# databricks/spark-deep-learning

Measured on AMD Instinct MI355X. Metric: images/sec, higher is better.
Workload: dtype bf16; 1 GPU; model=resnet50, global_batch=512, image=224, parallelism=dp1

## Files before the change

sparkdl/ops/csrc/batchnorm.hip:

```cpp

#include "common.hip.h"
#include "kernels.h"

namespace {

constexpr int kBlock = 256;
constexpr int kVec = 8;


__device__ __forceinline__ void bn_block_fold(
    float* lds_a, float* lds_b, const float* a, const float* b,
    int lane_col, int cols, float* out_a, float* out_b) {
  for (int c = threadIdx.x; c < cols; c += kBlock) {
    lds_a[c] = 0.f;
    lds_b[c] = 0.f;
  }
  __syncthreads();
#pragma unroll
  for (int j = 0; j < kVec; ++j) {
    atomicAdd(&lds_a[lane_col + j], a[j]);
    atomicAdd(&lds_b[lane_col + j], b[j]);
  }
  __syncthreads();
  for (int c = threadIdx.x; c < cols; c += kBlock) {
    atomicAdd(&out_a[c], lds_a[c]);
    atomicAdd(&out_b[c], lds_b[c]);
  }
}

__global__ __launch_bounds__(kBlock) void bn_stats_k(
    const short* __restrict__ x, float* __restrict__ scratch,
    long long rows, int cols) {
  __shared__ float lds[2 * 2048];
  const int tpr = cols / kVec;
  const int rpb = kBlock / min(tpr, kBlock);
  const int lane_col = (threadIdx.x % tpr) * kVec;
  const int row_off = threadIdx.x / tpr;

  float s[kVec] = {0.f}, ss[kVec] = {0.f};
  if (row_off < rpb) {
    for (long long r = (long long)blockIdx.x * rpb + row_off; r < rows;
         r += (long long)gridDim.x * rpb) {
      const short8 v = *(const short8*)(x + r * cols + lane_col);
#pragma unroll
      for (int j = 0; j < kVec; ++j) {
        const float f = bf2f(v[j]);
        s[j] += f;
        ss[j] += f * f;
      }
    }
  }
  bn_block_fold(lds, lds + cols, s, ss, lane_col, cols, scratch,
                scratch + cols);
}

__global__ void bn_finalize_k(
    const float* __restrict__ scratch, const float* __restrict__ gamma,
    const float* __restrict__ beta, float* __restrict__ running_mean,
    float* __restrict__ running_var, float* __restrict__ save_mean,
    float* __restrict__ save_rstd, float* __restrict__ scale,
    float* __restrict__ shift, long long rows, int cols, float momentum,
    float eps, int training) {
  const int c = blockIdx.x * blockDim.x + threadIdx.x;
  if (c >= cols) return;
  float mean, rstd;
  if (training) {
    mean = scratch[c] / rows;
    const float var = fmaxf(scratch[cols + c] / rows - mean * mean, 0.f);
    rstd = rsqrtf(var + eps);
    const float unbiased = rows > 1 ? var * rows / (rows - 1) : var;
    running_mean[c] += momentum * (mean - running_mean[c]);
    running_var[c] += momentum * (unbiased - running_var[c]);
    save_mean[c] = mean;
    save_rstd[c] = rstd;
  } else {
    mean = running_mean[c];
    rstd = rsqrtf(running_var[c] + eps);
    save_mean[c] = mean;
    save_rstd[c] = rstd;
  }
  const float sc = gamma[c] * rstd;
  scale[c] = sc;
  shift[c] = beta[c] - mean * sc;
}

template <bool RELU, bool RES>
__global__ __launch_bounds__(kBlock) void bn_apply_k(
    const short* __restrict__ x, const short* __restrict__ res,
    const float* __restrict__ scale, const float* __restrict__ shift,
    short* __restrict__ y, unsigned char* __restrict__ mask,
    long long rows, int cols) {
  const int tpr = cols / kVec;
  const int rpb = kBlock / min(tpr, kBlock);
  const int lane_col = (threadIdx.x % tpr) * kVec;
  const int row_off = threadIdx.x / tpr;
  if (row_off >= rpb) return;
  const float4v sc0 = *(const float4v*)(scale + lane_col);
  const float4v sc1 = *(const float4v*)(scale + lane_col + 4);
  const float4v sh0 = *(const float4v*)(shift + lane_col);
  const float4v sh1 = *(const float4v*)(shift + lane_col + 4);

  for (long long r = (long long)blockIdx.x * rpb + row_off; r < rows;
       r += (long long)gridDim.x * rpb) {
    const long long base = r * cols + lane_col;
    const short8 v = *(const short8*)(x + base);
    short8 o;
    unsigned char mbits = 0;
#pragma unroll
    for (int j = 0; j < kVec; ++j) {
      float f = bf2f(v[j]) * (j < 4 ? sc0[j] : sc1[j - 4]) +
                (j < 4 ? sh0[j] : sh1[j - 4]);
      if (RES) f += bf2f(res[base + j]);
      if (RELU) {
        if (f > 0.f) mbits |= (unsigned char)(1u << j);
        f = fmaxf(f, 0.f);
      }
      o[j] = f2bf(f);
    }
    *(short8*)(y + base) = o;
    if (RELU) mask[(r * cols + lane_col) / kVec] = mbits;
  }
}


template <bool RELU>
__global__ __launch_bounds__(kBlock) void bn_bwd_reduce_k(
    const short* __restrict__ x, const unsigned char* __restrict__ mask,
    const short* __restrict__ dy, const float* __restrict__ save_mean,
    const float* __restrict__ save_rstd, float* __restrict__ scratch,
    long long rows, int cols) {
  __shared__ float lds[2 * 2048];
  const int tpr = cols / kVec;
  const int rpb = kBlock / min(tpr, kBlock);
  const int lane_col = (threadIdx.x % tpr) * kVec;
  const int row_off = threadIdx.x / tpr;

  float s1[kVec] = {0.f}, s2[kVec] = {0.f};
  if (row_off < rpb) {
    const float4v m0 = *(const float4v*)(save_mean + lane_col);
    const float4v m1 = *(const float4v*)(save_mean + lane_col + 4);
    const float4v r0 = *(const float4v*)(save_rstd + lane_col);
    const float4v r1 = *(const float4v*)(save_rstd + lane_col + 4);
    for (long long r = (long long)blockIdx.x * rpb + row_off; r < rows;
         r += (long long)gridDim.x * rpb) {
      const long long base = r * cols + lane_col;
      const short8 xv = *(const short8*)(x + base);
      const short8 dv = *(const short8*)(dy + base);
      unsigned char mbits = 0xffu;
      if (RELU) mbits = mask[base / kVec];
#pragma unroll
      for (int j = 0; j < kVec; ++j) {
        float d = bf2f(dv[j]);
        if (RELU && !(mbits & (1u << j))) d = 0.f;
        const float mean = j < 4 ? m0[j] : m1[j - 4];
        const float rstd = j < 4 ? r0[j] : r1[j - 4];
        const float xh = (bf2f(xv[j]) - mean) * rstd;
        s1[j] += d;
        s2[j] += d * xh;
      }
    }
  }
  bn_block_fold(lds, lds + cols, s1, s2, lane_col, cols, scratch,
                scratch + cols);
}

__global__ void bn_bwd_finalize_k(
    const float* __restrict__ scratch, const float* __restrict__ gamma,
    const float* __restrict__ save_rstd, float* __restrict__ dgamma,
    float* __restrict__ dbeta, float* __restrict__ c1,
    float* __restrict__ c2, float* __restrict__ c3, long long rows,
    int cols, int training) {
  const int c = blockIdx.x * blockDim.x + threadIdx.x;
  if (c >= cols) return;
  const float sum_dym = scratch[c];
  const float sum_dymxh = scratch[cols + c];
  dgamma[c] = sum_dymxh;
  dbeta[c] = sum_dym;
  c1[c] = gamma[c] * save_rstd[c];
  if (training) {
    c2[c] = sum_dym / rows;
    c3[c] = sum_dymxh / rows;
  } else {
    c2[c] = 0.f;
    c3[c] = 0.f;
  }
}

template <bool RELU, bool RES>
__global__ __launch_bounds__(kBlock) void bn_bwd_apply_k(
    const short* __restrict__ x, const unsigned char* __restrict__ mask,
    const short* __restrict__ dy, const float* __restrict__ save_mean,
    const float* __restrict__ save_rstd, const float* __restrict__ c1,
    const float* __restrict__ c2, const float* __restrict__ c3,
    short* __restrict__ dx, short* __restrict__ dres, long long rows,
    int cols) {
  const int tpr = cols / kVec;
  const int rpb = kBlock / min(tpr, kBlock);
  const int lane_col = (threadIdx.x % tpr) * kVec;
  const int row_off = threadIdx.x / tpr;
  if (row_off >= rpb) return;
  const float4v m0 = *(const float4v*)(save_mean + lane_col);
  const float4v m1 = *(const float4v*)(save_mean + lane_col + 4);
  const float4v r0 = *(const float4v*)(save_rstd + lane_col);
  const float4v r1 = *(const float4v*)(save_rstd + lane_col + 4);
  const float4v a0 = *(const float4v*)(c1 + lane_col);
  const float4v a1 = *(const float4v*)(c1 + lane_col + 4);
  const float4v b0 = *(const float4v*)(c2 + lane_col);
  const float4v b1 = *(const float4v*)(c2 + lane_col + 4);
  const float4v g0 = *(const float4v*)(c3 + lane_col);
  const float4v g1 = *(const float4v*)(c3 + lane_col + 4);

  for (long long r = (long long)blockIdx.x * rpb + row_off; r < rows;
       r += (long long)gridDim.x * rpb) {
    const long long base = r * cols + lane_col;
    const short8 xv = *(const short8*)(x + base);
    const short8 dv = *(const short8*)(dy + base);
    unsigned char mbits = 0xffu;
    if (RELU) mbits = mask[base / kVec];
    short8 odx, odr;
#pragma unroll
    for (int j = 0; j < kVec; ++j) {
      float d = bf2f(dv[j]);
      if (RELU && !(mbits & (1u << j))) d = 0.f;
      const float mean = j < 4 ? m0[j] : m1[j - 4];
      const float rstd = j < 4 ? r0[j] : r1[j - 4];
      const float xh = (bf2f(xv[j]) - mean) * rstd;
      const float k1 = j < 4 ? a0[j] : a1[j - 4];
      const float k2 = j < 4 ? b0[j] : b1[j - 4];
      const float k3 = j < 4 ? g0[j] : g1[j - 4];
      odx[j] = f2bf(k1 * (d - k2 - xh * k3));
      if (RES) odr[j] = f2bf(d);
    }
    *(short8*)(dx + base) = odx;
    if (RES) *(short8*)(dres + base) = odr;
  }
}

int bn_grid(long long rows, int cols) {
  const int tpr = cols / kVec;
  const int rpb = kBlock / min(tpr, kBlock);
  long long blocks = (rows + rpb - 1) / rpb;
  return (int)min(blocks, 2048LL);
}

}

void launch_bn_fwd(const short* x, const short* res, const float* gamma,
                   const float* beta, float* running_mean,
                   float* running_var, float* save_mean, float* save_rstd,
                   float* scratch, short* y, unsigned char* mask,
                   long long rows, int cols, float momentum, float eps,
                   bool training, bool relu, hipStream_t stream) {
  const int grid = bn_grid(rows, cols);
  if (training)
    hipLaunchKernelGGL(bn_stats_k, dim3(grid), dim3(kBlock), 0, stream, x,
                       scratch, rows, cols);
  float* scale = scratch + 2 * cols;
  float* shift = scratch + 3 * cols;
  hipLaunchKernelGGL(bn_finalize_k, dim3((cols + 255) / 256), dim3(256), 0,
                     stream, scratch, gamma, beta, running_mean,
                     running_var, save_mean, save_rstd, scale, shift, rows,
                     cols, momentum, eps, (int)training);
  auto ap = relu ? (res ? bn_apply_k<true, true> : bn_apply_k<true, false>)
                 : (res ? bn_apply_k<false, true>
                        : bn_apply_k<false, false>);
  hipLaunchKernelGGL(ap, dim3(grid), dim3(kBlock), 0, stream, x, res,
                     scale, shift, y, mask, rows, cols);
}

void launch_bn_bwd(const short* x, const unsigned char* mask,
                   const short* dy, const float* gamma,
                   const float* save_mean, const float* save_rstd,
                   float* scratch, float* dgamma, float* dbeta, short* dx,
                   short* dres, long long rows, int cols, bool training,
                   bool relu, hipStream_t stream) {
  const int grid = bn_grid(rows, cols);
  auto rk = relu ? bn_bwd_reduce_k<true> : bn_bwd_reduce_k<false>;
  hipLaunchKernelGGL(rk, dim3(grid), dim3(kBlock), 0, stream, x, mask, dy,
                     save_mean, save_rstd, scratch, rows, cols);
  float* c1 = scratch + 2 * cols;
  float* c2 = scratch + 3 * cols;
  float* c3 = scratch + 4 * cols;
  hipLaunchKernelGGL(bn_bwd_finalize_k, dim3((cols + 255) / 256), dim3(256),
                     0, stream, scratch, gamma, save_rstd, dgamma, dbeta,
                     c1, c2, c3, rows, cols, (int)training);
  auto ak = relu ? (dres ? bn_bwd_apply_k<true, true>
                         : bn_bwd_apply_k<true, false>)
                 : (dres ? bn_bwd_apply_k<false, true>
                         : bn_bwd_apply_k<false, false>);
  hipLaunchKernelGGL(ak, dim3(grid), dim3(kBlock), 0, stream, x, mask, dy,
                     save_mean, save_rstd, c1, c2, c3, dx, dres, rows,
                     cols);
}
```

sparkdl/ops/csrc/bindings.cpp:

```cpp

#include <torch/extension.h>
#include <ATen/hip/impl/HIPStreamMasqueradingAsCUDA.h>
#include <ATen/hip/impl/HIPGuardImplMasqueradingAsCUDA.h>

#include <cmath>
#include <vector>

#include "kernels.h"

namespace {

using DeviceGuard = c10::hip::HIPGuardMasqueradingAsCUDA;

hipStream_t cur_stream() {
  return c10::hip::getCurrentHIPStreamMasqueradingAsCUDA().stream();
}

#define CHECK_BF16_CUDA(t)                                            \
  TORCH_CHECK((t).is_cuda(), #t " must be on GPU");                   \
  TORCH_CHECK((t).scalar_type() == at::kBFloat16, #t " must be bf16");\
  TORCH_CHECK((t).is_contiguous(), #t " must be contiguous")

#define CHECK_F32_CUDA(t)                                             \
  TORCH_CHECK((t).is_cuda(), #t " must be on GPU");                   \
  TORCH_CHECK((t).scalar_type() == at::kFloat, #t " must be fp32");   \
  TORCH_CHECK((t).is_contiguous(), #t " must be contiguous")

const short* bf_ptr(const at::Tensor& t) {
  return reinterpret_cast<const short*>(t.data_ptr<at::BFloat16>());
}
short* bf_ptr_mut(at::Tensor& t) {
  return reinterpret_cast<short*>(t.data_ptr<at::BFloat16>());
}


void fused_adamw_(const at::Tensor& chunks_blob, const at::Tensor& bmap,
                  int64_t nblocks, double lr, double beta1, double beta2,
                  double eps, double weight_decay, at::Tensor step_counter,
                  at::Tensor coeffs) {
  TORCH_CHECK(chunks_blob.is_cuda() && bmap.is_cuda());
  TORCH_CHECK(step_counter.is_cuda() &&
              step_counter.scalar_type() == at::kLong);
  TORCH_CHECK(coeffs.is_cuda() && coeffs.scalar_type() == at::kFloat &&
              coeffs.numel() >= 2);
  DeviceGuard guard(chunks_blob.device());
  launch_fused_adamw(
      reinterpret_cast<const TensorChunk*>(chunks_blob.data_ptr()),
      reinterpret_cast<const int2*>(bmap.data_ptr()), (int)nblocks,
      (float)lr, (float)beta1, (float)beta2, (float)eps,
      (float)weight_decay,
      reinterpret_cast<long long*>(step_counter.data_ptr<int64_t>()),
      coeffs.data_ptr<float>(), cur_stream());
}

void zero_grads_(const at::Tensor& chunks_blob, const at::Tensor& bmap,
                 int64_t nblocks) {
  TORCH_CHECK(chunks_blob.is_cuda() && bmap.is_cuda());
  DeviceGuard guard(chunks_blob.device());
  launch_zero_grads(
      reinterpret_cast<const TensorChunk*>(chunks_blob.data_ptr()),
      reinterpret_cast<const int2*>(bmap.data_ptr()), (int)nblocks,
      cur_stream());
}

void fused_sgd_(const at::Tensor& chunks_blob, const at::Tensor& bmap,
                int64_t nblocks, double lr, double momentum,
                double weight_decay, bool nesterov, bool first_step) {
  TORCH_CHECK(chunks_blob.is_cuda() && bmap.is_cuda());
  DeviceGuard guard(chunks_blob.device());
  launch_fused_sgd(
      reinterpret_cast<const TensorChunk*>(chunks_blob.data_ptr()),
      reinterpret_cast<const int2*>(bmap.data_ptr()), (int)nblocks,
      (float)lr, (float)momentum, (float)weight_decay, nesterov,
      first_step, cur_stream());
}


std::vector<at::Tensor> layernorm_fwd(const at::Tensor& x,
                                      const at::Tensor& gamma,
                                      const at::Tensor& beta, double eps) {
  CHECK_BF16_CUDA(x);
  CHECK_F32_CUDA(gamma);
  CHECK_F32_CUDA(beta);
  DeviceGuard guard(x.device());
  const int cols = (int)x.size(-1);
  const int rows = (int)(x.numel() / cols);
  TORCH_CHECK(gamma.numel() == cols && beta.numel() == cols);

  auto y = at::empty_like(x);
  auto f32 = x.options().dtype(at::kFloat);
  auto mean = at::empty({rows}, f32);
  auto rstd = at::empty({rows}, f32);
  launch_layernorm_fwd(bf_ptr(x), gamma.data_ptr<float>(),
                       beta.data_ptr<float>(), bf_ptr_mut(y),
                       mean.data_ptr<float>(), rstd.data_ptr<float>(),
                       rows, cols, (float)eps, cur_stream());
  return {y, mean, rstd};
}

std::vector<at::Tensor> layernorm_bwd(const at::Tensor& x,
                                      const at::Tensor& dy,
                                      const at::Tensor& gamma,
                                      const at::Tensor& mean,
                                      const at::Tensor& rstd) {
  CHECK_BF16_CUDA(x);
  CHECK_BF16_CUDA(dy);
  CHECK_F32_CUDA(gamma);
  DeviceGuard guard(x.device());
  const int cols = (int)x.size(-1);
  const int rows = (int)(x.numel() / cols);
  TORCH_CHECK(cols <= 8192, "layernorm_bwd LDS partials support cols<=8192");

  auto dx = at::empty_like(x);
  auto f32 = x.options().dtype(at::kFloat);
  const int blocks = layernorm_bwd_part_rows(rows);
  const int ws_rows = blocks * 4;
  auto dgamma_part = at::empty({ws_rows, cols}, f32);
  auto dbeta_part = at::empty({ws_rows, cols}, f32);
  auto dgamma = at::zeros({cols}, f32);
  auto dbeta = at::zeros({cols}, f32);
  launch_layernorm_bwd(bf_ptr(x), bf_ptr(dy), gamma.data_ptr<float>(),
                       mean.data_ptr<float>(), rstd.data_ptr<float>(),
                       bf_ptr_mut(dx), dgamma_part.data_ptr<float>(),
                       dbeta_part.data_ptr<float>(), blocks, rows, cols,
                       cur_stream());
  launch_layernorm_reduce_parts(
      dgamma_part.data_ptr<float>(), dbeta_part.data_ptr<float>(),
      dgamma.data_ptr<float>(), dbeta.data_ptr<float>(), ws_rows, cols,
      cur_stream());
  return {dx, dgamma, dbeta};
}


std::vector<at::Tensor> bn_fwd(const at::Tensor& x,
                               const c10::optional<at::Tensor>& res,
                               const at::Tensor& gamma,
                               const at::Tensor& beta,
                               at::Tensor running_mean,
                               at::Tensor running_var, double momentum,
                               double eps, bool training, bool relu) {
  CHECK_BF16_CUDA(x);
  CHECK_F32_CUDA(gamma);
  CHECK_F32_CUDA(beta);
  DeviceGuard guard(x.device());
  const int cols = (int)x.size(-1);
  const long long rows = x.numel() / cols;
  TORCH_CHECK(cols % 8 == 0 && cols <= 2048,
              "bn_fwd requires cols%8==0 and cols<=2048 (NHWC channels)");
  const short* res_ptr = nullptr;
  if (res.has_value()) {
    CHECK_BF16_CUDA(res.value());
    TORCH_CHECK(res->sizes() == x.sizes());
    res_ptr = bf_ptr(res.value());
  }
  auto f32 = x.options().dtype(at::kFloat);
  auto y = at::empty_like(x);
  auto save_mean = at::empty({cols}, f32);
  auto save_rstd = at::empty({cols}, f32);
  auto scratch = at::zeros({5 * cols}, f32);
  at::Tensor mask;
  unsigned char* mask_ptr = nullptr;
  if (relu) {
    mask = at::empty({rows * cols / 8}, x.options().dtype(at::kByte));
    mask_ptr = mask.data_ptr<unsigned char>();
  } else {
    mask = at::empty({0}, x.options().dtype(at::kByte));
  }
  launch_bn_fwd(bf_ptr(x), res_ptr, gamma.data_ptr<float>(),
                beta.data_ptr<float>(), running_mean.data_ptr<float>(),
                running_var.data_ptr<float>(), save_mean.data_ptr<float>(),
                save_rstd.data_ptr<float>(), scratch.data_ptr<float>(),
                bf_ptr_mut(y), mask_ptr, rows, cols, (float)momentum,
                (float)eps, training, relu, cur_stream());
  return {y, save_mean, save_rstd, mask};
}

std::vector<at::Tensor> bn_bwd(const at::Tensor& x,
                               const at::Tensor& mask,
                               const at::Tensor& dy,
                               const at::Tensor& gamma,
                               const at::Tensor& save_mean,
                               const at::Tensor& save_rstd, bool training,
                               bool relu, bool needs_dres) {
  CHECK_BF16_CUDA(x);
  CHECK_BF16_CUDA(dy);
  CHECK_F32_CUDA(gamma);
  DeviceGuard guard(x.device());
  const int cols = (int)x.size(-1);
  const long long rows = x.numel() / cols;
  TORCH_CHECK(!relu || mask.numel() == rows * cols / 8,
              "relu backward needs the forward's activation mask");
  auto f32 = x.options().dtype(at::kFloat);
  auto dx = at::empty_like(x);
  auto dgamma = at::empty({cols}, f32);
  auto dbeta = at::empty({cols}, f32);
  auto scratch = at::zeros({5 * cols}, f32);
  at::Tensor dres;
  short* dres_ptr = nullptr;
  if (needs_dres) {
    dres = at::empty_like(x);
    dres_ptr = bf_ptr_mut(dres);
  }
  launch_bn_bwd(bf_ptr(x),
                relu ? mask.data_ptr<unsigned char>() : nullptr,
                bf_ptr(dy), gamma.data_ptr<float>(),
                save_mean.data_ptr<float>(), save_rstd.data_ptr<float>(),
                scratch.data_ptr<float>(), dgamma.data_ptr<float>(),
                dbeta.data_ptr<float>(), bf_ptr_mut(dx), dres_ptr, rows,
                cols, training, relu, cur_stream());
  if (needs_dres) return {dx, dgamma, dbeta, dres};
  return {dx, dgamma, dbeta};
}


at::Tensor bias_gelu_fwd(const at::Tensor& x, const at::Tensor& bias) {
  CHECK_BF16_CUDA(x);
  CHECK_F32_CUDA(bias);
  DeviceGuard guard(x.device());
  const int cols = (int)x.size(-1);
  const long long rows = x.numel() / cols;
  TORCH_CHECK(bias.numel() == cols);
  auto y = at::empty_like(x);
  launch_bias_gelu_fwd(bf_ptr(x), bias.data_ptr<float>(), bf_ptr_mut(y),
                       rows, cols, cur_stream());
  return y;
}

std::vector<at::Tensor> bias_gelu_bwd(const at::Tensor& x,
                                      const at::Tensor& bias,
                                      const at::Tensor& dy) {
  CHECK_BF16_CUDA(x);
  CHECK_BF16_CUDA(dy);
  CHECK_F32_CUDA(bias);
  DeviceGuard guard(x.device());
  const int cols = (int)x.size(-1);
  const long long rows = x.numel() / cols;
  TORCH_CHECK(cols <= 16384, "bias_gelu_bwd LDS partials support cols<=16384");
  auto dx = at::empty_like(x);
  auto dbias = at::zeros({cols}, x.options().dtype(at::kFloat));
  launch_bias_gelu_bwd(bf_ptr(x), bias.data_ptr<float>(), bf_ptr(dy),
                       bf_ptr_mut(dx), dbias.data_ptr<float>(), rows, cols,
                       cur_stream());
  return {dx, dbias};
}


std::vector<at::Tensor> gemm_bias_act(const at::Tensor& A,
                                      const at::Tensor& W,
                                      const c10::optional<at::Tensor>& bias,
                                      int64_t act, bool save_z) {
  CHECK_BF16_CUDA(A);
  CHECK_BF16_CUDA(W);
  TORCH_CHECK(A.dim() == 2 && W.dim() == 2 && A.size(1) == W.size(1));
  const int M = (int)A.size(0), K = (int)A.size(1), N = (int)W.size(0);
  TORCH_CHECK(gemm_bias_act_supported(M, N, K),
              "gemm_bias_act requires K % 64 == 0");
  const float* bias_ptr = nullptr;
  if (bias.has_value()) {
    CHECK_F32_CUDA(bias.value());
    TORCH_CHECK(bias->numel() == N);
    bias_ptr = bias->data_ptr<float>();
  }
  DeviceGuard guard(A.device());
  auto C = at::empty({M, N}, A.options());
  at::Tensor Z;
  short* z_ptr = nullptr;
  if (save_z && act != 0) {
    Z = at::empty({M, N}, A.options());
    z_ptr = bf_ptr_mut(Z);
  }
  launch_gemm_bias_act(bf_ptr(A), bf_ptr(W), bias_ptr, bf_ptr_mut(C),
                       z_ptr, M, N, K, (int)act, cur_stream());
  if (z_ptr) return {C, Z};
  return {C};
}

at::Tensor gemm_stream(const at::Tensor& A, const at::Tensor& W) {
  CHECK_BF16_CUDA(A);
  CHECK_BF16_CUDA(W);
  TORCH_CHECK(A.dim() == 2 && W.dim() == 2 && A.size(1) == W.size(1));
  const long long M = A.size(0);
  const int K = (int)A.size(1), N = (int)W.size(0);
  TORCH_CHECK(gemm_stream_supported(M, N, K),
              "gemm_stream requires K in {64,128,256} and N % 64 == 0");
  DeviceGuard guard(A.device());
  auto C = at::empty({M, N}, A.options());
  launch_gemm_stream(bf_ptr(A), bf_ptr(W), bf_ptr_mut(C), M, N, K,
                     cur_stream());
  return C;
}


static const long long* seed_ptr(const c10::optional<at::Tensor>& seed) {
  if (!seed.has_value()) return nullptr;
  TORCH_CHECK(seed->is_cuda() && seed->scalar_type() == at::kLong &&
              seed->numel() >= 1);
  return reinterpret_cast<const long long*>(seed->data_ptr<int64_t>());
}

std::vector<at::Tensor> attn_fwd(const at::Tensor& Q, const at::Tensor& K,
                                 const at::Tensor& V, double dropout_p,
                                 const c10::optional<at::Tensor>& seed) {
  CHECK_BF16_CUDA(Q);
  CHECK_BF16_CUDA(K);
  CHECK_BF16_CUDA(V);
  TORCH_CHECK(Q.dim() == 3 && Q.size(2) == 64 && Q.sizes() == K.sizes() &&
                  Q.sizes() == V.sizes(),
              "attn_fwd expects [BH, S, 64] bf16 q/k/v");
  const int BH = (int)Q.size(0), S = (int)Q.size(1);
  TORCH_CHECK(S % 64 == 0, "attn_fwd requires S % 64 == 0");
  TORCH_CHECK(dropout_p == 0.0 || seed.has_value(),
              "dropout needs a seed tensor");
  DeviceGuard guard(Q.device());
  auto O = at::empty_like(Q);
  auto LSE = at::empty({BH, S}, Q.options().dtype(at::kFloat));
  auto VT = at::empty({BH, 64, S}, Q.options());
  launch_attn_pretranspose(bf_ptr(V), bf_ptr_mut(VT), BH, S, 1, 64,
                           cur_stream());
  launch_attn_fwd(bf_ptr(Q), bf_ptr(K), bf_ptr(VT), bf_ptr_mut(O),
                  LSE.data_ptr<float>(), seed_ptr(seed), BH, S, 1, 64,
                  64, (float)dropout_p, cur_stream());
  return {O, LSE};
}

std::vector<at::Tensor> attn_fwd_packed(
    const at::Tensor& qkv, double dropout_p,
    const c10::optional<at::Tensor>& seed) {
  CHECK_BF16_CUDA(qkv);
  TORCH_CHECK(qkv.dim() == 5 && qkv.size(2) == 3 && qkv.size(4) == 64 &&
                  qkv.is_contiguous(),
              "attn_fwd_packed expects contiguous [B,S,3,H,64] bf16");
  const int B = (int)qkv.size(0), S = (int)qkv.size(1),
            H = (int)qkv.size(3);
  TORCH_CHECK(S % 64 == 0, "attn requires S % 64 == 0");
  TORCH_CHECK(dropout_p == 0.0 || seed.has_value());
  DeviceGuard guard(qkv.device());
  auto O = at::empty({B, S, H * 64}, qkv.options());
  auto LSE = at::empty({B * H, S}, qkv.options().dtype(at::kFloat));
  const short* base = bf_ptr(qkv);
  auto VT = at::empty({B * H, 64, S}, qkv.options());
  launch_attn_pretranspose(base + (long long)2 * H * 64, bf_ptr_mut(VT),
                           B * H, S, H, 3 * H * 64, cur_stream());
  launch_attn_fwd(base, base + (long long)H * 64, bf_ptr(VT),
                  bf_ptr_mut(O), LSE.data_ptr<float>(), seed_ptr(seed),
                  B * H, S, H, 3 * H * 64, H * 64, (float)dropout_p,
                  cur_stream());
  return {O, LSE};
}

std::vector<at::Tensor> attn_bwd(const at::Tensor& Q, const at::Tensor& K,
                                 const at::Tensor& V, const at::Tensor& dO,
                                 const at::Tensor& LSE,
                                 const at::Tensor& Drow, double dropout_p,
                                 const c10::optional<at::Tensor>& seed) {
  CHECK_BF16_CUDA(Q);
  CHECK_BF16_CUDA(dO);
  CHECK_F32_CUDA(LSE);
  CHECK_F32_CUDA(Drow);
  const int BH = (int)Q.size(0), S = (int)Q.size(1);
  DeviceGuard guard(Q.device());
  auto dQ = at::empty_like(Q);
  auto dK = at::empty_like(K);
  auto dV = at::empty_like(V);
  auto T3 = at::empty({3, BH, 64, S}, Q.options());
  short* qt = bf_ptr_mut(T3);
  short* dot = qt + (long long)BH * 64 * S;
  short* ktt = dot + (long long)BH * 64 * S;
  launch_attn_pretranspose(bf_ptr(Q), qt, BH, S, 1, 64, cur_stream());
  launch_attn_pretranspose(bf_ptr(dO), dot, BH, S, 1, 64, cur_stream());
  launch_attn_pretranspose(bf_ptr(K), ktt, BH, S, 1, 64, cur_stream());
  launch_attn_bwd(bf_ptr(Q), bf_ptr(K), bf_ptr(V), bf_ptr(dO), qt, dot,
                  ktt, LSE.data_ptr<float>(), Drow.data_ptr<float>(),
                  bf_ptr_mut(dQ), bf_ptr_mut(dK), bf_ptr_mut(dV),
                  seed_ptr(seed), BH, S, 1, 64, 64, 64, (float)dropout_p,
                  cur_stream());
  return {dQ, dK, dV};
}

at::Tensor attn_bwd_packed(const at::Tensor& qkv, const at::Tensor& dO,
                           const at::Tensor& LSE, const at::Tensor& Drow,
                           double dropout_p,
                           const c10::optional<at::Tensor>& seed) {
  CHECK_BF16_CUDA(qkv);
  CHECK_BF16_CUDA(dO);
  CHECK_F32_CUDA(LSE);
  CHECK_F32_CUDA(Drow);
  TORCH_CHECK(qkv.dim() == 5 && qkv.is_contiguous() &&
              dO.is_contiguous());
  const int B = (int)qkv.size(0), S = (int)qkv.size(1),
            H = (int)qkv.size(3);
  DeviceGuard guard(qkv.device());
  auto dqkv = at::empty_like(qkv);
  const short* base = bf_ptr(qkv);
  short* gbase = bf_ptr_mut(dqkv);
  const int BH = B * H;
  auto T3 = at::empty({3, BH, 64, S}, qkv.options());
  short* qt = bf_ptr_mut(T3);
  short* dot = qt + (long long)BH * 64 * S;
  short* ktt = dot + (long long)BH * 64 * S;
  launch_attn_pretranspose(base, qt, BH, S, H, 3 * H * 64, cur_stream());
  launch_attn_pretranspose(bf_ptr(dO), dot, BH, S, H, H * 64,
                           cur_stream());
  launch_attn_pretranspose(base + (long long)H * 64, ktt, BH, S, H,
                           3 * H * 64, cur_stream());
  launch_attn_bwd(base, base + (long long)H * 64,
                  base + (long long)2 * H * 64, bf_ptr(dO), qt, dot, ktt,
                  LSE.data_ptr<float>(), Drow.data_ptr<float>(), gbase,
                  gbase + (long long)H * 64,
                  gbase + (long long)2 * H * 64, seed_ptr(seed), BH, S,
                  H, 3 * H * 64, H * 64, 3 * H * 64, (float)dropout_p,
                  cur_stream());
  return dqkv;
}

at::Tensor wgrad_splitk(const at::Tensor& dZ, const at::Tensor& X) {
  CHECK_BF16_CUDA(dZ);
  CHECK_BF16_CUDA(X);
  TORCH_CHECK(dZ.dim() == 2 && X.dim() == 2 && dZ.size(0) == X.size(0));
  const long long M = dZ.size(0);
  const int N = (int)dZ.size(1), K = (int)X.size(1);
  TORCH_CHECK(wgrad_splitk_supported(M, N, K),
              "wgrad_splitk requires N%256==0, K%128==0, M%64==0");
  DeviceGuard guard(dZ.device());
  auto dW = at::empty({N, K}, dZ.options().dtype(at::kFloat));
  launch_wgrad_splitk(bf_ptr(dZ), bf_ptr(X), dW.data_ptr<float>(), M, N,
                      K, cur_stream());
  return dW;
}

at::Tensor transpose_bf16(const at::Tensor& X) {
  CHECK_BF16_CUDA(X);
  TORCH_CHECK(X.dim() == 2 && X.is_contiguous());
  DeviceGuard guard(X.device());
  const int R = (int)X.size(0), C = (int)X.size(1);
  auto Y = at::empty({C, R}, X.options());
  launch_transpose_bf16(bf_ptr(X), bf_ptr_mut(Y), R, C, cur_stream());
  return Y;
}


at::Tensor gbt_histogram(const at::Tensor& B, const at::Tensor& g,
                         const at::Tensor& h, const at::Tensor& row_list,
                         const at::Tensor& bmap, int64_t n_nodes) {
  TORCH_CHECK(B.is_cuda() && B.scalar_type() == at::kByte &&
              B.is_contiguous());
  CHECK_F32_CUDA(g);
  CHECK_F32_CUDA(h);
  TORCH_CHECK(row_list.is_cuda() && row_list.scalar_type() == at::kInt);
  TORCH_CHECK(bmap.is_cuda() && bmap.scalar_type() == at::kInt &&
              bmap.size(-1) == 4);
  DeviceGuard guard(B.device());
  const int F = (int)B.size(1);
  TORCH_CHECK(F % 8 == 0, "feature dim must be padded to a multiple of 8");
  auto hist = at::zeros({n_nodes, F, 256, 2},
                        B.options().dtype(at::kFloat));
  launch_gbt_histogram(
      B.data_ptr<unsigned char>(), g.data_ptr<float>(),
      h.data_ptr<float>(), row_list.data_ptr<int>(),
      reinterpret_cast<const int4*>(bmap.data_ptr<int>()),
      (int)(bmap.numel() / 4), F, hist.data_ptr<float>(), cur_stream());
  return hist;
}

}

PYBIND11_MODULE(TORCH_EXTENSION_NAME, m) {
  m.doc() = "sparkdl MI355X-native kernels (gfx950)";
  m.def("fused_adamw_", &fused_adamw_, "Fused multi-tensor AdamW step");
  m.def("fused_sgd_", &fused_sgd_, "Fused multi-tensor SGD step");
  m.def("zero_grads_", &zero_grads_, "Zero all grads in a chunk table");
  m.def("gemm_bias_act", &gemm_bias_act, "MFMA GEMM + bias(+GELU) (N6)");
  m.def("transpose_bf16", &transpose_bf16, "bf16 2D transpose (dgrad W^T)");
  m.def("gemm_stream", &gemm_stream,
        "Streaming tall-skinny GEMM (1x1 convs)");
  m.def("wgrad_splitk", &wgrad_splitk,
        "Split-M wgrad GEMM (tr_b16 fragment path)");
  m.def("attn_fwd", &attn_fwd, "Flash attention fwd (D=64, bf16)");
  m.def("attn_bwd", &attn_bwd, "Flash attention bwd (dQ/dK/dV)");
  m.def("attn_fwd_packed", &attn_fwd_packed,
        "Flash attention fwd over the packed qkv buffer");
  m.def("attn_bwd_packed", &attn_bwd_packed,
        "Flash attention bwd -> packed dqkv");
  m.def("gbt_histogram", &gbt_histogram, "GBT g/h histogram (N7)");
  m.def("bn_fwd", &bn_fwd, "Fused BatchNorm(+add)(+ReLU) fwd (bf16 NHWC)");
  m.def("bn_bwd", &bn_bwd, "Fused BatchNorm(+add)(+ReLU) bwd (bf16 NHWC)");
  m.def("layernorm_fwd", &layernorm_fwd, "LayerNorm forward (bf16)");
  m.def("layernorm_bwd", &layernorm_bwd, "LayerNorm backward (bf16)");
  m.def("bias_gelu_fwd", &bias_gelu_fwd, "Fused bias+GELU forward (bf16)");
  m.def("bias_gelu_bwd", &bias_gelu_bwd, "Fused bias+GELU backward (bf16)");
  m.attr("_chunk_elems") = kOptChunk;
}
```

sparkdl/ops/csrc/kernels.h:

```cpp
#pragma once

#include <hip/hip_runtime.h>
#include <cstdint>

struct TensorChunk {
  float* p;
  const float* g;
  float* m;
  float* v;
  long long n;
  short* pl;
};

constexpr int kOptChunk = 16384;

void launch_fused_adamw(const TensorChunk* chunks, const int2* bmap,
                        int nblocks, float lr, float beta1, float beta2,
                        float eps, float weight_decay,
                        long long* step_counter, float* coeffs,
                        hipStream_t stream);

void launch_fused_sgd(const TensorChunk* chunks, const int2* bmap,
                      int nblocks, float lr, float momentum,
                      float weight_decay, bool nesterov, bool first_step,
                      hipStream_t stream);

void launch_layernorm_fwd(const short* x, const float* gamma,
                          const float* beta, short* y, float* save_mean,
                          float* save_rstd, int rows, int cols, float eps,
                          hipStream_t stream);

void launch_layernorm_bwd(const short* x, const short* dy,
                          const float* gamma, const float* save_mean,
                          const float* save_rstd, short* dx,
                          float* dgamma_part, float* dbeta_part,
                          int part_rows, int rows, int cols,
                          hipStream_t stream);

int layernorm_bwd_part_rows(int rows);

void launch_layernorm_reduce_parts(const float* dgamma_part,
                                   const float* dbeta_part, float* dgamma,
                                   float* dbeta, int part_rows, int cols,
                                   hipStream_t stream);

void launch_bias_gelu_fwd(const short* x, const float* bias, short* y,
                          long long rows, int cols, hipStream_t stream);

void launch_bias_gelu_bwd(const short* x, const float* bias,
                          const short* dy, short* dx, float* dbias,
                          long long rows, int cols, hipStream_t stream);

void launch_bn_fwd(const short* x, const short* res, const float* gamma,
                   const float* beta, float* running_mean,
                   float* running_var, float* save_mean, float* save_rstd,
                   float* scratch, short* y, unsigned char* mask,
                   long long rows, int cols, float momentum, float eps,
                   bool training, bool relu, hipStream_t stream);

void launch_bn_bwd(const short* x, const unsigned char* mask,
                   const short* dy, const float* gamma,
                   const float* save_mean, const float* save_rstd,
                   float* scratch, float* dgamma, float* dbeta, short* dx,
                   short* dres, long long rows, int cols, bool training,
                   bool relu, hipStream_t stream);

void launch_gemm_bias_act(const short* A, const short* W,
                          const float* bias, short* C, short* Z, int M,
                          int N, int K, int act, hipStream_t stream);
bool gemm_bias_act_supported(int M, int N, int K);

void launch_gemm_stream(const short* A, const short* W, short* C,
                        long long M, int N, int K, hipStream_t stream);
bool gemm_stream_supported(long long M, int N, int K);

void launch_wgrad_splitk(const short* dZ, const short* X, float* dW,
                         long long M, int N, int K, hipStream_t stream);
bool wgrad_splitk_supported(long long M, int N, int K);

void launch_transpose_bf16(const short* X, short* Y, int R, int C,
                           hipStream_t stream);

void launch_attn_pretranspose(const short* X, short* T, int BH, int S,
                              int H, int rs, hipStream_t stream);
void launch_attn_fwd(const short* Q, const short* K, const short* VT,
                     short* O, float* LSE, const long long* seed, int BH,
                     int S, int H, int rs, int ors, float dropout_p,
                     hipStream_t stream);
void launch_attn_bwd(const short* Q, const short* K, const short* V,
                     const short* dO, const short* QT, const short* DOT,
                     const short* KT, const float* LSE, const float* Drow,
                     short* dQ, short* dK, short* dV,
                     const long long* seed, int BH, int S, int H, int rs,
                     int ors, int grs, float dropout_p,
                     hipStream_t stream);

void launch_gbt_histogram(const unsigned char* B, const float* g,
                          const float* h, const int* row_list,
                          const int4* bmap, int nblocks, int F,
                          float* hist, hipStream_t stream);

void launch_zero_grads(const TensorChunk* chunks, const int2* bmap,
                       int nblocks, hipStream_t stream);
```

Before: 8714 images/s.

## Replace atomic BN reductions with per-block slabs and parallel finalize

```diff
diff --git a/sparkdl/ops/csrc/batchnorm.hip b/sparkdl/ops/csrc/batchnorm.hip
--- a/sparkdl/ops/csrc/batchnorm.hip
+++ b/sparkdl/ops/csrc/batchnorm.hip
@@ -6,32 +6,95 @@
 
 constexpr int kBlock = 256;
 constexpr int kVec = 8;
-
+constexpr int kUnroll = 2;
+constexpr int kFoldFloats = kBlock * 2 * kVec;
+constexpr int kFinCh = 4;
+
+
+__device__ __forceinline__ void bn_store_pair(
+    float* p, int cols, const float (&a)[kVec], const float (&b)[kVec]) {
+  *(float4v*)(p) = float4v{a[0], a[1], a[2], a[3]};
+  *(float4v*)(p + 4) = float4v{a[4], a[5], a[6], a[7]};
+  *(float4v*)(p + cols) = float4v{b[0], b[1], b[2], b[3]};
+  *(float4v*)(p + cols + 4) = float4v{b[4], b[5], b[6], b[7]};
+}
 
 __device__ __forceinline__ void bn_block_fold(
-    float* lds_a, float* lds_b, const float* a, const float* b,
-    int lane_col, int cols, float* out_a, float* out_b) {
-  for (int c = threadIdx.x; c < cols; c += kBlock) {
-    lds_a[c] = 0.f;
-    lds_b[c] = 0.f;
+    float* lds, float (&a)[kVec], float (&b)[kVec], int rpb, int row_off,
+    int lane_col, int cols, float* __restrict__ slab_row) {
+  const bool active = row_off < rpb;
+  float* mine = lds + (size_t)row_off * 2 * cols + lane_col;
+  if (active) bn_store_pair(mine, cols, a, b);
+  int s = 1;
+  while (s < rpb) s <<= 1;
+  int n = rpb;
+  for (s >>= 1; s >= 1; s >>= 1) {
+    __syncthreads();
+    if (row_off < s && row_off + s < n) {
+      const float* peer = mine + (size_t)s * 2 * cols;
+      const float4v pa0 = *(const float4v*)(peer);
+      const float4v pa1 = *(const float4v*)(peer + 4);
+      const float4v pb0 = *(const float4v*)(peer + cols);
+      const float4v pb1 = *(const float4v*)(peer + cols + 4);
+#pragma unroll
+      for (int j = 0; j < 4; ++j) {
+        a[j] += pa0[j];
+        a[j + 4] += pa1[j];
+        b[j] += pb0[j];
+        b[j + 4] += pb1[j];
+      }
+      if (s > 1) bn_store_pair(mine, cols, a, b);
+    }
+    n = min(n, s);
+  }
+  if (row_off == 0) bn_store_pair(slab_row + lane_col, cols, a, b);
+}
+
+__device__ __forceinline__ void bn_slab_sum(
+    const float* __restrict__ slab, int G, int cols, int blk, float* red,
+    float& sum_a, float& sum_b) {
+  const int c = blk * kFinCh + threadIdx.x % kFinCh;
+  float sa = 0.f, sb = 0.f;
+#pragma unroll 4
+  for (int g = threadIdx.x / kFinCh; g < G; g += kBlock / kFinCh) {
+    const float* row = slab + (size_t)g * 2 * cols;
+    sa += row[c];
+    sb += row[cols + c];
+  }
+#pragma unroll
+  for (int off = kFinCh; off < WAVE; off <<= 1) {
+    sa += __shfl_xor(sa, off, WAVE);
+    sb += __shfl_xor(sb, off, WAVE);
+  }
+  const int lane = threadIdx.x % WAVE;
+  const int wid = threadIdx.x / WAVE;
+  if (lane < kFinCh) {
+    red[wid * 2 * kFinCh + lane] = sa;
+    red[wid * 2 * kFinCh + kFinCh + lane] = sb;
   }
   __syncthreads();
-#pragma unroll
-  for (int j = 0; j < kVec; ++j) {
-    atomicAdd(&lds_a[lane_col + j], a[j]);
-    atomicAdd(&lds_b[lane_col + j], b[j]);
-  }
-  __syncthreads();
-  for (int c = threadIdx.x; c < cols; c += kBlock) {
-    atomicAdd(&out_a[c], lds_a[c]);
-    atomicAdd(&out_b[c], lds_b[c]);
-  }
-}
-
+  sum_a = 0.f;
+  sum_b = 0.f;
+  if (threadIdx.x < kFinCh) {
+#pragma unroll
+    for (int w = 0; w < kBlock / WAVE; ++w) {
+      sum_a += red[w * 2 * kFinCh + threadIdx.x];
+      sum_b += red[w * 2 * kFinCh + kFinCh + threadIdx.x];
+    }
+  }
+}
+
+__device__ __forceinline__ int bn_fin_block() {
+  const int nb = gridDim.x;
+  if (nb % 8) return blockIdx.x;
+  return (blockIdx.x % 8) * (nb / 8) + blockIdx.x / 8;
+}
+
+template <int U>
 __global__ __launch_bounds__(kBlock) void bn_stats_k(
-    const short* __restrict__ x, float* __restrict__ scratch,
+    const short* __restrict__ x, float* __restrict__ slab,
     long long rows, int cols) {
-  __shared__ float lds[2 * 2048];
+  __shared__ __attribute__((aligned(16))) float lds[kFoldFloats];
   const int tpr = cols / kVec;
   const int rpb = kBlock / min(tpr, kBlock);
   const int lane_col = (threadIdx.x % tpr) * kVec;
@@ -39,8 +102,24 @@
 
   float s[kVec] = {0.f}, ss[kVec] = {0.f};
   if (row_off < rpb) {
-    for (long long r = (long long)blockIdx.x * rpb + row_off; r < rows;
-         r += (long long)gridDim.x * rpb) {
+    const long long stride = (long long)gridDim.x * rpb;
+    long long r = (long long)blockIdx.x * rpb + row_off;
+    for (; r + (U - 1) * stride < rows; r += U * stride) {
+      short8 v[U];
+#pragma unroll
+      for (int u = 0; u < U; ++u)
+        v[u] = *(const short8*)(x + (r + u * stride) * cols + lane_col);
+#pragma unroll
+      for (int u = 0; u < U; ++u) {
+#pragma unroll
+        for (int j = 0; j < kVec; ++j) {
+          const float f = bf2f(v[u][j]);
+          s[j] += f;
+          ss[j] += f * f;
+        }
+      }
+    }
+    for (; r < rows; r += stride) {
       const short8 v = *(const short8*)(x + r * cols + lane_col);
 #pragma unroll
       for (int j = 0; j < kVec; ++j) {
@@ -50,23 +129,27 @@
       }
     }
   }
-  bn_block_fold(lds, lds + cols, s, ss, lane_col, cols, scratch,
-                scratch + cols);
-}
-
-__global__ void bn_finalize_k(
-    const float* __restrict__ scratch, const float* __restrict__ gamma,
+  bn_block_fold(lds, s, ss, rpb, row_off, lane_col, cols,
+                slab + (size_t)blockIdx.x * 2 * cols);
+}
+
+__global__ __launch_bounds__(kBlock) void bn_finalize_k(
+    const float* __restrict__ slab, int G, const float* __restrict__ gamma,
     const float* __restrict__ beta, float* __restrict__ running_mean,
     float* __restrict__ running_var, float* __restrict__ save_mean,
     float* __restrict__ save_rstd, float* __restrict__ scale,
     float* __restrict__ shift, long long rows, int cols, float momentum,
     float eps, int training) {
-  const int c = blockIdx.x * blockDim.x + threadIdx.x;
-  if (c >= cols) return;
+  __shared__ float red[kBlock / WAVE * 2 * kFinCh];
+  float sum = 0.f, sumsq = 0.f;
+  const int blk = bn_fin_block();
+  if (training) bn_slab_sum(slab, G, cols, blk, red, sum, sumsq);
+  if (threadIdx.x >= kFinCh) return;
+  const int c = blk * kFinCh + threadIdx.x;
   float mean, rstd;
   if (training) {
-    mean = scratch[c] / rows;
-    const float var = fmaxf(scratch[cols + c] / rows - mean * mean, 0.f);
+    mean = sum / rows;
+    const float var = fmaxf(sumsq / rows - mean * mean, 0.f);
     rstd = rsqrtf(var + eps);
     const float unbiased = rows > 1 ? var * rows / (rows - 1) : var;
     running_mean[c] += momentum * (mean - running_mean[c]);
@@ -123,13 +206,13 @@
 }
 
 
-template <bool RELU>
+template <bool RELU, int U>
 __global__ __launch_bounds__(kBlock) void bn_bwd_reduce_k(
     const short* __restrict__ x, const unsigned char* __restrict__ mask,
     const short* __restrict__ dy, const float* __restrict__ save_mean,
-    const float* __restrict__ save_rstd, float* __restrict__ scratch,
+    const float* __restrict__ save_rstd, float* __restrict__ slab,
     long long rows, int cols) {
-  __shared__ float lds[2 * 2048];
+  __shared__ __attribute__((aligned(16))) float lds[kFoldFloats];
   const int tpr = cols / kVec;
   const int rpb = kBlock / min(tpr, kBlock);
   const int lane_col = (threadIdx.x % tpr) * kVec;
@@ -141,13 +224,8 @@
     const float4v m1 = *(const float4v*)(save_mean + lane_col + 4);
     const float4v r0 = *(const float4v*)(save_rstd + lane_col);
     const float4v r1 = *(const float4v*)(save_rstd + lane_col + 4);
-    for (long long r = (long long)blockIdx.x * rpb + row_off; r < rows;
-         r += (long long)gridDim.x * rpb) {
-      const long long base = r * cols + lane_col;
-      const short8 xv = *(const short8*)(x + base);
-      const short8 dv = *(const short8*)(dy + base);
-      unsigned char mbits = 0xffu;
-      if (RELU) mbits = mask[base / kVec];
+    auto accum = [&](const short8& xv, const short8& dv,
+                     unsigned char mbits) {
 #pragma unroll
       for (int j = 0; j < kVec; ++j) {
         float d = bf2f(dv[j]);
@@ -158,22 +236,48 @@
         s1[j] += d;
         s2[j] += d * xh;
       }
-    }
-  }
-  bn_block_fold(lds, lds + cols, s1, s2, lane_col, cols, scratch,
-                scratch + cols);
-}
-
-__global__ void bn_bwd_finalize_k(
-    const float* __restrict__ scratch, const float* __restrict__ gamma,
+    };
+    const long long stride = (long long)gridDim.x * rpb;
+    long long r = (long long)blockIdx.x * rpb + row_off;
+    for (; r + (U - 1) * stride < rows; r += U * stride) {
+      short8 xv[U], dv[U];
+      unsigned char mb[U];
+#pragma unroll
+      for (int u = 0; u < U; ++u) {
+        const long long base = (r + u * stride) * cols + lane_col;
+        xv[u] = *(const short8*)(x + base);
+        dv[u] = *(const short8*)(dy + base);
+        mb[u] = 0xffu;
+        if (RELU) mb[u] = mask[base / kVec];
+      }
+#pragma unroll
+      for (int u = 0; u < U; ++u) accum(xv[u], dv[u], mb[u]);
+    }
+    for (; r < rows; r += stride) {
+      const long long base = r * cols + lane_col;
+      const short8 xv = *(const short8*)(x + base);
+      const short8 dv = *(const short8*)(dy + base);
+      unsigned char mbits = 0xffu;
+      if (RELU) mbits = mask[base / kVec];
+      accum(xv, dv, mbits);
+    }
+  }
+  bn_block_fold(lds, s1, s2, rpb, row_off, lane_col, cols,
+                slab + (size_t)blockIdx.x * 2 * cols);
+}
+
+__global__ __launch_bounds__(kBlock) void bn_bwd_finalize_k(
+    const float* __restrict__ slab, int G, const float* __restrict__ gamma,
     const float* __restrict__ save_rstd, float* __restrict__ dgamma,
     float* __restrict__ dbeta, float* __restrict__ c1,
     float* __restrict__ c2, float* __restrict__ c3, long long rows,
     int cols, int training) {
-  const int c = blockIdx.x * blockDim.x + threadIdx.x;
-  if (c >= cols) return;
-  const float sum_dym = scratch[c];
-  const float sum_dymxh = scratch[cols + c];
+  __shared__ float red[kBlock / WAVE * 2 * kFinCh];
+  float sum_dym, sum_dymxh;
+  const int blk = bn_fin_block();
+  bn_slab_sum(slab, G, cols, blk, red, sum_dym, sum_dymxh);
+  if (threadIdx.x >= kFinCh) return;
+  const int c = blk * kFinCh + threadIdx.x;
   dgamma[c] = sum_dymxh;
   dbeta[c] = sum_dym;
   c1[c] = gamma[c] * save_rstd[c];
@@ -245,6 +349,18 @@
 
 }
 
+int bn_reduce_blocks(long long rows, int cols) {
+  const int tpr = cols / kVec;
+  const int rpb = kBlock / min(tpr, kBlock);
+  const long long row_blocks = (rows + rpb - 1) / rpb;
+  const long long g = max(256LL, min(512LL, rows / 64));
+  return (int)max(1LL, min(row_blocks, g));
+}
+
+long long bn_scratch_floats(long long rows, int cols) {
+  return (long long)bn_reduce_blocks(rows, cols) * 2 * cols + 3LL * cols;
+}
+
 void launch_bn_fwd(const short* x, const short* res, const float* gamma,
                    const float* beta, float* running_mean,
                    float* running_var, float* save_mean, float* save_rstd,
@@ -252,13 +368,14 @@
                    long long rows, int cols, float momentum, float eps,
                    bool training, bool relu, hipStream_t stream) {
   const int grid = bn_grid(rows, cols);
+  const int G = bn_reduce_blocks(rows, cols);
   if (training)
-    hipLaunchKernelGGL(bn_stats_k, dim3(grid), dim3(kBlock), 0, stream, x,
-                       scratch, rows, cols);
-  float* scale = scratch + 2 * cols;
-  float* shift = scratch + 3 * cols;
-  hipLaunchKernelGGL(bn_finalize_k, dim3((cols + 255) / 256), dim3(256), 0,
-                     stream, scratch, gamma, beta, running_mean,
+    hipLaunchKernelGGL(bn_stats_k<kUnroll>, dim3(G), dim3(kBlock), 0,
+                       stream, x, scratch, rows, cols);
+  float* scale = scratch + (size_t)G * 2 * cols;
+  float* shift = scale + cols;
+  hipLaunchKernelGGL(bn_finalize_k, dim3(cols / kFinCh), dim3(kBlock), 0,
+                     stream, scratch, G, gamma, beta, running_mean,
                      running_var, save_mean, save_rstd, scale, shift, rows,
                      cols, momentum, eps, (int)training);
   auto ap = relu ? (res ? bn_apply_k<true, true> : bn_apply_k<true, false>)
@@ -275,14 +392,16 @@
                    short* dres, long long rows, int cols, bool training,
                    bool relu, hipStream_t stream) {
   const int grid = bn_grid(rows, cols);
-  auto rk = relu ? bn_bwd_reduce_k<true> : bn_bwd_reduce_k<false>;
-  hipLaunchKernelGGL(rk, dim3(grid), dim3(kBlock), 0, stream, x, mask, dy,
+  const int G = bn_reduce_blocks(rows, cols);
+  auto rk = relu ? bn_bwd_reduce_k<true, kUnroll>
+                 : bn_bwd_reduce_k<false, kUnroll>;
+  hipLaunchKernelGGL(rk, dim3(G), dim3(kBlock), 0, stream, x, mask, dy,
                      save_mean, save_rstd, scratch, rows, cols);
-  float* c1 = scratch + 2 * cols;
-  float* c2 = scratch + 3 * cols;
-  float* c3 = scratch + 4 * cols;
-  hipLaunchKernelGGL(bn_bwd_finalize_k, dim3((cols + 255) / 256), dim3(256),
-                     0, stream, scratch, gamma, save_rstd, dgamma, dbeta,
+  float* c1 = scratch + (size_t)G * 2 * cols;
+  float* c2 = c1 + cols;
+  float* c3 = c2 + cols;
+  hipLaunchKernelGGL(bn_bwd_finalize_k, dim3(cols / kFinCh), dim3(kBlock),
+                     0, stream, scratch, G, gamma, save_rstd, dgamma, dbeta,
                      c1, c2, c3, rows, cols, (int)training);
   auto ak = relu ? (dres ? bn_bwd_apply_k<true, true>
                          : bn_bwd_apply_k<true, false>)
diff --git a/sparkdl/ops/csrc/bindings.cpp b/sparkdl/ops/csrc/bindings.cpp
--- a/sparkdl/ops/csrc/bindings.cpp
+++ b/sparkdl/ops/csrc/bindings.cpp
@@ -157,7 +157,7 @@
   auto y = at::empty_like(x);
   auto save_mean = at::empty({cols}, f32);
   auto save_rstd = at::empty({cols}, f32);
-  auto scratch = at::zeros({5 * cols}, f32);
+  auto scratch = at::empty({bn_scratch_floats(rows, cols)}, f32);
   at::Tensor mask;
   unsigned char* mask_ptr = nullptr;
   if (relu) {
@@ -194,7 +194,7 @@
   auto dx = at::empty_like(x);
   auto dgamma = at::empty({cols}, f32);
   auto dbeta = at::empty({cols}, f32);
-  auto scratch = at::zeros({5 * cols}, f32);
+  auto scratch = at::empty({bn_scratch_floats(rows, cols)}, f32);
   at::Tensor dres;
   short* dres_ptr = nullptr;
   if (needs_dres) {
diff --git a/sparkdl/ops/csrc/kernels.h b/sparkdl/ops/csrc/kernels.h
--- a/sparkdl/ops/csrc/kernels.h
+++ b/sparkdl/ops/csrc/kernels.h
@@ -51,6 +51,9 @@
                           const short* dy, short* dx, float* dbias,
                           long long rows, int cols, hipStream_t stream);
 
+int bn_reduce_blocks(long long rows, int cols);
+long long bn_scratch_floats(long long rows, int cols);
+
 void launch_bn_fwd(const short* x, const short* res, const float* gamma,
                    const float* beta, float* running_mean,
                    float* running_var, float* save_mean, float* save_rstd,
```

After: 9520 images/s (median of 6 runs). 9.2% higher.
